# Siverteh/semantic-slam-master

Hardware: AMD Instinct MI355X
Metric: frames/sec extract+match on TUM 640x480; match-index bit-exact vs CPU ref (higher is better)
Workload: dtype f32

## Files before the change

semantic-slam-master_amd/csrc/resample.hip:

```cpp
#include <math.h>

#include <algorithm>

#include "common.h"

namespace {

typedef unsigned u32x4 __attribute__((ext_vector_type(4)));
typedef unsigned u32x2 __attribute__((ext_vector_type(2)));

constexpr int PREC = 22;
constexpr int TX = 64, TY = 16, MAXR = 64;

__device__ __forceinline__ int clip8(int v) {
    v >>= PREC;
    return v < 0 ? 0 : (v > 255 ? 255 : v);
}

__global__ __launch_bounds__(256) void preprocess_kernel(const uint8_t *__restrict__ img, int h, int w, int size,
                                                          const int *__restrict__ bh, const int *__restrict__ ch, int ksh,
                                                          const int *__restrict__ bv, const int *__restrict__ cv, int ksv,
                                                          float *__restrict__ out) {
    __shared__ uint8_t tmp[MAXR][TX][3];
    __shared__ float lut[3][256];
    const int tid = threadIdx.x;
    const long long f = blockIdx.z;
    const int x0 = blockIdx.x * TX, y0 = blockIdx.y * TY;
    const int ty1 = min(y0 + TY, size) - 1;
    const int rmin = bv[2 * y0], rmax = bv[2 * ty1] + bv[2 * ty1 + 1];
    const int nrows = rmax - rmin;
    const uint8_t *src = img + f * h * w * 3;
    {
        const float mean[3] = {0.485f, 0.456f, 0.406f}, sd[3] = {0.229f, 0.224f, 0.225f};
#pragma unroll
        for (int c = 0; c < 3; c++) lut[c][tid] = ((float)tid / 255.0f - mean[c]) / sd[c];
    }
    for (int it = tid; it < nrows * TX; it += 256) {
        const int rr = it / TX, xx = it % TX;
        const int ox = x0 + xx;
        if (ox < size) {
            const int xmin = bh[2 * ox], xn = bh[2 * ox + 1];
            const int *k = ch + (long long)ox * ksh;
            const uint8_t *p = src + ((long long)(rmin + rr) * w + xmin) * 3;
            int s0 = 1 << (PREC - 1), s1 = s0, s2 = s0;
            for (int t = 0; t < xn; t++) {
                const int kk = k[t];
                s0 += p[3 * t] * kk;
                s1 += p[3 * t + 1] * kk;
                s2 += p[3 * t + 2] * kk;
            }
            tmp[rr][xx][0] = (uint8_t)clip8(s0);
            tmp[rr][xx][1] = (uint8_t)clip8(s1);
            tmp[rr][xx][2] = (uint8_t)clip8(s2);
        }
    }
    __syncthreads();
    const long long plane = (long long)size * size;
    for (int it = tid; it < TY * TX * 3; it += 256) {
        const int c = it / (TY * TX), rem = it % (TY * TX), yy = rem / TX, xx = rem % TX;
        const int oy = y0 + yy, ox = x0 + xx;
        if (oy < size && ox < size) {
            const int ymin = bv[2 * oy] - rmin, yn = bv[2 * oy + 1];
            const int *k = cv + (long long)oy * ksv;
            int s = 1 << (PREC - 1);
            for (int t = 0; t < yn; t++) s += tmp[ymin + t][xx][c] * k[t];
            out[(f * 3 + c) * plane + (long long)oy * size + ox] = lut[c][clip8(s)];
        }
    }
}

template <int TAPS, int TYT, int MAXRT, bool PATCH = false>
__global__ __launch_bounds__(256) void preprocess_fast_kernel(const uint8_t *__restrict__ img, unsigned total_bytes, int h, int w,
                                                               int size, const int *__restrict__ bh, const int *__restrict__ ch,
                                                               int ksh, const int *__restrict__ bv, const int *__restrict__ cv,
                                                               int ksv, float *__restrict__ out, int gx, int tiles, int n_frames) {
    __shared__ unsigned tmp[MAXRT][TX];
    __shared__ float lut[3][256];
    const int tid = threadIdx.x;
    const int bq = blockIdx.x >> 3;
    const unsigned f = (unsigned)((bq / tiles) * 8 + (blockIdx.x & 7));
    if ((int)f >= n_frames) return;
    const int tl = bq % tiles;
    const int x0 = (tl % gx) * TX, y0 = (tl / gx) * TYT;
    const int ty1 = min(y0 + TYT, size) - 1;
    const int rmin = bv[2 * y0], rmax = bv[2 * ty1] + bv[2 * ty1 + 1];
    const int nrows = rmax - rmin;
    const __amdgpu_buffer_rsrc_t irs =
        __builtin_amdgcn_make_buffer_rsrc(const_cast<uint8_t *>(img), 0, (int)((total_bytes + 3u) & ~3u), 0x00020000);
    {
        const float mean[3] = {0.485f, 0.456f, 0.406f}, sd[3] = {0.229f, 0.224f, 0.225f};
#pragma unroll
        for (int c = 0; c < 3; c++) lut[c][tid] = ((float)tid / 255.0f - mean[c]) / sd[c];
    }
    const int xx = tid & (TX - 1), q = __builtin_amdgcn_readfirstlane(tid >> 6);
    const int ox = min(x0 + xx, size - 1);
    {
        const int xmin = bh[2 * ox], xn = bh[2 * ox + 1];
        constexpr int NW = (3 * TAPS + 3 + 3) / 4;
        int kh[TAPS];
#pragma unroll
        for (int t = 0; t < TAPS; t++) kh[t] = t < xn ? ch[ox * ksh + t] : 0;
        const unsigned col0 = f * (unsigned)(h * w * 3) + (unsigned)(rmin * w + xmin) * 3u;
        const unsigned rstride = (unsigned)w * 3u;
        constexpr int RB = 3;
        for (int rr0 = q; rr0 < nrows; rr0 += 4 * RB) {
            unsigned wds[RB][8];
            int shv[RB];
#pragma unroll
            for (int i = 0; i < RB; i++) {
                const int rr = min(rr0 + 4 * i, nrows - 1);
                const unsigned b0 = col0 + (unsigned)rr * rstride;
                const int a0 = (int)(b0 & ~3u);
                shv[i] = (int)(b0 & 3u);
                const u32x4 lo = __builtin_amdgcn_raw_buffer_load_b128(irs, a0, 0, 0);
                wds[i][0] = lo[0], wds[i][1] = lo[1], wds[i][2] = lo[2], wds[i][3] = lo[3];
                if constexpr (NW == 5) wds[i][4] = __builtin_amdgcn_raw_buffer_load_b32(irs, a0, 16, 0);
                if constexpr (NW == 6) {
                    const u32x2 hi = __builtin_amdgcn_raw_buffer_load_b64(irs, a0, 16, 0);
                    wds[i][4] = hi[0], wds[i][5] = hi[1];
                }
            }
#pragma unroll
            for (int i = 0; i < RB; i++) {
                const int rr = rr0 + 4 * i;
                if (rr >= nrows) break;
                const int sh = shv[i];
                unsigned al[NW];
#pragma unroll
                for (int j = 0; j < NW - 1; j++) al[j] = __builtin_amdgcn_alignbyte(wds[i][j + 1], wds[i][j], sh);
                al[NW - 1] = wds[i][NW - 1] >> (8 * sh);
                int s0 = 1 << (PREC - 1), s1 = s0, s2 = s0;
#pragma unroll
                for (int t = 0; t < TAPS; t++) {
                    const int o = 3 * t;
                    const int r8 = (al[o >> 2] >> (8 * (o & 3))) & 255;
                    const int g8 = (al[(o + 1) >> 2] >> (8 * ((o + 1) & 3))) & 255;
                    const int b8 = (al[(o + 2) >> 2] >> (8 * ((o + 2) & 3))) & 255;
                    s0 += __mul24(r8, kh[t]);
                    s1 += __mul24(g8, kh[t]);
                    s2 += __mul24(b8, kh[t]);
                }
                tmp[rr][xx] = (unsigned)clip8(s0) | ((unsigned)clip8(s1) << 8) | ((unsigned)clip8(s2) << 16);
            }
        }
    }
    __syncthreads();
    const long long plane = (long long)size * size;
    if (x0 + xx < size) {
#pragma unroll
        for (int j = 0; j < TYT / 4; j++) {
            const int oy = y0 + q * (TYT / 4) + j;
            if (oy < size) {
                const int ymin = bv[2 * oy] - rmin, yn = bv[2 * oy + 1];
                const int *k = cv + oy * ksv;
                int s0 = 1 << (PREC - 1), s1 = s0, s2 = s0;
                for (int t = 0; t < yn; t++) {
                    const unsigned p = tmp[ymin + t][xx];
                    const int kk = k[t];
                    s0 += __mul24((int)(p & 255), kk);
                    s1 += __mul24((int)((p >> 8) & 255), kk);
                    s2 += __mul24((int)((p >> 16) & 255), kk);
                }
                if constexpr (PATCH) {
                    const int G = size >> 4, ox_ = x0 + xx;
                    __bf16 *o = reinterpret_cast<__bf16 *>(out) +
                                (((long long)f * G + (oy >> 4)) * G + (ox_ >> 4)) * 768 + (oy & 15) * 16 + (ox_ & 15);
                    o[0] = (__bf16)lut[0][clip8(s0)];
                    o[256] = (__bf16)lut[1][clip8(s1)];
                    o[512] = (__bf16)lut[2][clip8(s2)];
                } else {
                    float *o = out + (long long)f * 3 * plane + (long long)oy * size + (x0 + xx);
                    o[0] = lut[0][clip8(s0)];
                    o[plane] = lut[1][clip8(s1)];
                    o[2 * plane] = lut[2][clip8(s2)];
                }
            }
        }
    }
}

__global__ __launch_bounds__(256) void intensity_kernel(const uint8_t *__restrict__ img, int h, int w, int size,
                                                         const int *__restrict__ bh, const int *__restrict__ ch, int ksh,
                                                         const int *__restrict__ bv, const int *__restrict__ cv, int ksv,
                                                         const float *__restrict__ kp_pixel, int K, long long total,
                                                         float *__restrict__ out) {
    const long long i = (long long)blockIdx.x * 256 + threadIdx.x;
    if (i >= total) return;
    const long long f = i / K;
    const uint8_t *src = img + f * h * w * 3;
    int X = (int)__builtin_rintf(kp_pixel[2 * i]), Y = (int)__builtin_rintf(kp_pixel[2 * i + 1]);
    X = min(max(X, 0), size - 1);
    Y = min(max(Y, 0), size - 1);
    const int xmin = bh[2 * X], xn = bh[2 * X + 1], ymin = bv[2 * Y], yn = bv[2 * Y + 1];
    const int *kh = ch + (long long)X * ksh, *kv = cv + (long long)Y * ksv;
    int a0 = 1 << (PREC - 1), a1 = a0, a2 = a0;
    for (int ry = 0; ry < yn; ry++) {
        const uint8_t *p = src + ((long long)(ymin + ry) * w + xmin) * 3;
        int s0 = 1 << (PREC - 1), s1 = s0, s2 = s0;
        for (int t = 0; t < xn; t++) {
            const int kk = kh[t];
            s0 += p[3 * t] * kk;
            s1 += p[3 * t + 1] * kk;
            s2 += p[3 * t + 2] * kk;
        }
        const int kk = kv[ry];
        a0 += clip8(s0) * kk;
        a1 += clip8(s1) * kk;
        a2 += clip8(s2) * kk;
    }
    const int R = clip8(a0), Gc = clip8(a1), B = clip8(a2);
    const int L = (R * 19595 + Gc * 38470 + B * 7471 + 0x8000) >> 16;
    out[i] = (float)L / 255.0f;
}

double filt_bilinear(double x) {
    if (x < 0.0) x = -x;
    return x < 1.0 ? 1.0 - x : 0.0;
}
double filt_bicubic(double x) {
    const double a = -0.5;
    if (x < 0.0) x = -x;
    if (x < 1.0) return ((a + 2.0) * x - (a + 3.0)) * x * x + 1;
    if (x < 2.0) return (((x - 5) * x + 8) * x - 4) * a;
    return 0.0;
}

}

extern "C" int sslam_resample_table_host(int in_size, int out_size, int filter, int32_t *bounds, int32_t *coefs,
                                         int coefs_capacity) {
    if (in_size <= 0 || out_size <= 0 || !bounds || !coefs || filter < 0 || filter > 1) return SSLAM_E_INVALID;
    double (*fn)(double) = filter ? filt_bicubic : filt_bilinear;
    const double scale = (double)in_size / out_size;
    double filterscale = scale;
    if (filterscale < 1.0) filterscale = 1.0;
    const double support = (filter ? 2.0 : 1.0) * filterscale;
    const int ksize = (int)ceil(support) * 2 + 1;
    if (ksize > SSLAM_MAX_TAPS) return SSLAM_E_UNSUPPORTED;
    if ((long long)ksize * out_size > coefs_capacity) return SSLAM_E_INVALID;
    double k[SSLAM_MAX_TAPS];
    for (int xx = 0; xx < out_size; xx++) {
        const double center = 0.0 + (xx + 0.5) * scale;
        const double ss = 1.0 / filterscale;
        double ww = 0.0;
        int xmin = (int)(center - support + 0.5);
        if (xmin < 0) xmin = 0;
        int xmax = (int)(center + support + 0.5);
        if (xmax > in_size) xmax = in_size;
        xmax -= xmin;
        int x;
        for (x = 0; x < xmax; x++) {
            const double wgt = fn((x + xmin - center + 0.5) * ss);
            k[x] = wgt;
            ww += wgt;
        }
        for (x = 0; x < xmax; x++)
            if (ww != 0.0) k[x] /= ww;
        for (; x < ksize; x++) k[x] = 0;
        for (x = 0; x < ksize; x++)
            coefs[(long long)xx * ksize + x] =
                k[x] < 0 ? (int32_t)(-0.5 + k[x] * (1 << PREC)) : (int32_t)(0.5 + k[x] * (1 << PREC));
        bounds[2 * xx] = xmin;
        bounds[2 * xx + 1] = xmax;
    }
    return ksize;
}

template <bool PATCH>
static int preprocess_launch(const uint8_t *img, int n, int h, int w, int size, const int32_t *bounds_h, const int32_t *coefs_h,
                             int ksize_h, const int32_t *bounds_v, const int32_t *coefs_v, int ksize_v, void *out_v, void *stream) {
    if (!img || !bounds_h || !coefs_h || !bounds_v || !coefs_v || !out_v || n <= 0 || h <= 0 || w <= 0 || size <= 0)
        return SSLAM_E_INVALID;
    if (ksize_h <= 0 || ksize_v <= 0 || ksize_h > SSLAM_MAX_TAPS || ksize_v > SSLAM_MAX_TAPS) return SSLAM_E_INVALID;
    if (PATCH && size % 16) return SSLAM_E_INVALID;
    if (sslam_misaligned(4, bounds_h, coefs_h, bounds_v, coefs_v) || sslam_misaligned(PATCH ? 2 : 4, out_v)) return SSLAM_E_INVALID;
    if ((long long)(TY * (long long)h + size - 1) / size + ksize_v + 2 > MAXR) return SSLAM_E_UNSUPPORTED;
    const bool tall = (32LL * h + size - 1) / size + ksize_v + 2 <= 64;
    const long long fbytes = (long long)h * w * 3;
    if (fbytes > 0x7fffffffLL) return SSLAM_E_UNSUPPORTED;
    int per_group = (int)std::min<long long>(65535, std::max<long long>(1, 0xfffffff0LL / fbytes));
    if ((fbytes & 3) && per_group >= 4) per_group &= ~3;
    for (int n0 = 0; n0 < n; n0 += per_group) {
        const int ng = std::min(per_group, n - n0);
        const uint8_t *gi = img + (long long)n0 * fbytes;
        const bool aligned = !((uintptr_t)gi & 3);
        float *go = PATCH ? reinterpret_cast<float *>(reinterpret_cast<__bf16 *>(out_v) + (long long)n0 * 3 * size * size)
                          : reinterpret_cast<float *>(out_v) + (long long)n0 * 3 * size * size;
        const unsigned gbytes = (unsigned)(ng * fbytes);
        const dim3 grid((size + TX - 1) / TX, (size + TY - 1) / TY, ng);
        const int gx = (size + TX - 1) / TX, tiles_t = gx * ((size + 31) / 32), tiles_s = gx * ((size + TY - 1) / TY);
        const long long nb_t = (long long)((ng + 7) / 8) * 8 * tiles_t, nb_s = (long long)((ng + 7) / 8) * 8 * tiles_s;
        if (nb_t > 0x7fffffffLL || nb_s > 0x7fffffffLL) return SSLAM_E_UNSUPPORTED;
#define FAST(T)                                                                                                        \
    {                                                                                                                  \
        if (tall)                                                                                                      \
            hipLaunchKernelGGL((preprocess_fast_kernel<T, 32, 64, PATCH>), dim3((unsigned)nb_t), dim3(256), 0, (hipStream_t)stream, gi, gbytes, h, w, \
                               size, bounds_h, coefs_h, ksize_h, bounds_v, coefs_v, ksize_v, go, gx, tiles_t, ng);     \
        else                                                                                                           \
            hipLaunchKernelGGL((preprocess_fast_kernel<T, TY, MAXR, PATCH>), dim3((unsigned)nb_s), dim3(256), 0, (hipStream_t)stream, gi, gbytes, h, w, \
                               size, bounds_h, coefs_h, ksize_h, bounds_v, coefs_v, ksize_v, go, gx, tiles_s, ng);     \
    }
        if (ksize_h <= 3 && aligned)
            FAST(3)
        else if (ksize_h <= 5 && aligned)
            FAST(5)
        else if (ksize_h <= 7 && aligned)
            FAST(7)
        else if (PATCH)
            return SSLAM_E_UNSUPPORTED;
        else
            hipLaunchKernelGGL(preprocess_kernel, grid, dim3(256), 0, (hipStream_t)stream, gi, h, w, size, bounds_h, coefs_h,
                               ksize_h, bounds_v, coefs_v, ksize_v, go);
#undef FAST
    }
    SSLAM_CHECK_LAUNCH();
    return SSLAM_OK;
}

extern "C" int sslam_preprocess_u8(const uint8_t *img, int n, int h, int w, int size, const int32_t *bounds_h,
                                   const int32_t *coefs_h, int ksize_h, const int32_t *bounds_v, const int32_t *coefs_v,
                                   int ksize_v, float *out_chw, void *stream) {
    return preprocess_launch<false>(img, n, h, w, size, bounds_h, coefs_h, ksize_h, bounds_v, coefs_v, ksize_v, out_chw, stream);
}

extern "C" int sslam_preprocess_u8_patches(const uint8_t *img, int n, int h, int w, int size, const int32_t *bounds_h,
                                           const int32_t *coefs_h, int ksize_h, const int32_t *bounds_v, const int32_t *coefs_v,
                                           int ksize_v, void *out_patches_bf16, void *stream) {
    return preprocess_launch<true>(img, n, h, w, size, bounds_h, coefs_h, ksize_h, bounds_v, coefs_v, ksize_v, out_patches_bf16, stream);
}

extern "C" int sslam_keypoint_intensity(const uint8_t *img, int n, int h, int w, int size, const int32_t *bounds_h,
                                        const int32_t *coefs_h, int ksize_h, const int32_t *bounds_v, const int32_t *coefs_v,
                                        int ksize_v, const float *kp_pixel, int K, float *out, void *stream) {
    if (!img || !bounds_h || !coefs_h || !bounds_v || !coefs_v || !kp_pixel || !out || n <= 0 || h <= 0 || w <= 0 ||
        size <= 0 || K <= 0)
        return SSLAM_E_INVALID;
    if (sslam_misaligned(4, bounds_h, coefs_h, bounds_v, coefs_v, kp_pixel, out)) return SSLAM_E_INVALID;
    const long long total = (long long)n * K;
    hipLaunchKernelGGL(intensity_kernel, dim3((unsigned)((total + 255) / 256)), dim3(256), 0, (hipStream_t)stream, img, h, w,
                       size, bounds_h, coefs_h, ksize_h, bounds_v, coefs_v, ksize_v, kp_pixel, K, total, out);
    SSLAM_CHECK_LAUNCH();
    return SSLAM_OK;
}
```

Measured before the change: 58200.

## Add templated buffer-load keypoint intensity kernel and nontemporal preprocess stores

Adds a templated intensity kernel for small filter sizes. It fetches each source row with wide raw buffer loads, unpacks the bytes with alignbyte, and fully unrolls both filter passes, replacing per-byte global loads inside dynamic loops. The preprocess kernel gains asm barriers that keep the batched row loads in registers so they stay issued ahead of use, and its f32 output now uses nontemporal stores to avoid polluting the cache. The fast path is taken only when kernel sizes, image alignment and sizes allow; otherwise the old kernel still runs. This adds code size and template variants.

```diff
diff --git a/semantic-slam-master_amd/csrc/resample.hip b/semantic-slam-master_amd/csrc/resample.hip
--- a/semantic-slam-master_amd/csrc/resample.hip
+++ b/semantic-slam-master_amd/csrc/resample.hip
@@ -120,6 +120,10 @@
                     wds[i][4] = hi[0], wds[i][5] = hi[1];
                 }
             }
+#pragma unroll
+            for (int i = 0; i < RB; i++)
+#pragma unroll
+                for (int j = 0; j < NW; j++) asm volatile("" : "+v"(wds[i][j]));
 #pragma unroll
             for (int i = 0; i < RB; i++) {
                 const int rr = rr0 + 4 * i;
@@ -170,9 +174,9 @@
                     o[512] = (__bf16)lut[2][clip8(s2)];
                 } else {
                     float *o = out + (long long)f * 3 * plane + (long long)oy * size + (x0 + xx);
-                    o[0] = lut[0][clip8(s0)];
-                    o[plane] = lut[1][clip8(s1)];
-                    o[2 * plane] = lut[2][clip8(s2)];
+                    __builtin_nontemporal_store(lut[0][clip8(s0)], o);
+                    __builtin_nontemporal_store(lut[1][clip8(s1)], o + plane);
+                    __builtin_nontemporal_store(lut[2][clip8(s2)], o + 2 * plane);
                 }
             }
         }
@@ -210,6 +214,70 @@
     }
     const int R = clip8(a0), Gc = clip8(a1), B = clip8(a2);
     const int L = (R * 19595 + Gc * 38470 + B * 7471 + 0x8000) >> 16;
+    out[i] = (float)L / 255.0f;
+}
+
+template <int TAPS, int VT>
+__global__ __launch_bounds__(256) void intensity_fast_kernel(const uint8_t *__restrict__ img, unsigned total_bytes, int h, int w,
+                                                              int size, const int *__restrict__ bh, const int *__restrict__ ch,
+                                                              int ksh, const int *__restrict__ bv, const int *__restrict__ cv,
+                                                              int ksv, const float *__restrict__ kp_pixel, int K, int total,
+                                                              float *__restrict__ out) {
+    const int i = blockIdx.x * 256 + threadIdx.x;
+    if (i >= total) return;
+    const unsigned f = (unsigned)i / (unsigned)K;
+    const __amdgpu_buffer_rsrc_t irs =
+        __builtin_amdgcn_make_buffer_rsrc(const_cast<uint8_t *>(img), 0, (int)((total_bytes + 3u) & ~3u), 0x00020000);
+    int X = (int)__builtin_rintf(kp_pixel[2 * (size_t)i]), Y = (int)__builtin_rintf(kp_pixel[2 * (size_t)i + 1]);
+    X = min(max(X, 0), size - 1);
+    Y = min(max(Y, 0), size - 1);
+    const int xmin = bh[2 * X], xn = bh[2 * X + 1], ymin = bv[2 * Y], yn = bv[2 * Y + 1];
+    constexpr int NW = (3 * TAPS + 3 + 3) / 4;
+    const unsigned col0 = f * (unsigned)(h * w * 3) + (unsigned)(ymin * w + xmin) * 3u;
+    const unsigned rstride = (unsigned)w * 3u;
+    unsigned wds[VT][8];
+#pragma unroll
+    for (int ry = 0; ry < VT; ry++) {
+#pragma unroll
+        for (int j = 0; j < NW; j++) wds[ry][j] = 0;
+        if (ry < yn) {
+            const int a0 = (int)((col0 + (unsigned)ry * rstride) & ~3u);
+            const u32x4 lo = __builtin_amdgcn_raw_buffer_load_b128(irs, a0, 0, 0);
+            wds[ry][0] = lo[0], wds[ry][1] = lo[1], wds[ry][2] = lo[2], wds[ry][3] = lo[3];
+            if constexpr (NW == 5) wds[ry][4] = __builtin_amdgcn_raw_buffer_load_b32(irs, a0, 16, 0);
+            if constexpr (NW == 6) {
+                const u32x2 hi = __builtin_amdgcn_raw_buffer_load_b64(irs, a0, 16, 0);
+                wds[ry][4] = hi[0], wds[ry][5] = hi[1];
+            }
+        }
+    }
+    int kh[TAPS], kv[VT];
+#pragma unroll
+    for (int t = 0; t < TAPS; t++) kh[t] = t < xn ? ch[X * ksh + min(t, ksh - 1)] : 0;
+#pragma unroll
+    for (int t = 0; t < VT; t++) kv[t] = t < yn ? cv[Y * ksv + min(t, ksv - 1)] : 0;
+    int a0 = 1 << (PREC - 1), a1 = a0, a2 = a0;
+#pragma unroll
+    for (int ry = 0; ry < VT; ry++) {
+        const int sh = (int)((col0 + (unsigned)ry * rstride) & 3u);
+        unsigned al[NW];
+#pragma unroll
+        for (int j = 0; j < NW - 1; j++) al[j] = __builtin_amdgcn_alignbyte(wds[ry][j + 1], wds[ry][j], sh);
+        al[NW - 1] = wds[ry][NW - 1] >> (8 * sh);
+        int s0 = 1 << (PREC - 1), s1 = s0, s2 = s0;
+#pragma unroll
+        for (int t = 0; t < TAPS; t++) {
+            const int o = 3 * t;
+            s0 += __mul24((int)((al[o >> 2] >> (8 * (o & 3))) & 255), kh[t]);
+            s1 += __mul24((int)((al[(o + 1) >> 2] >> (8 * ((o + 1) & 3))) & 255), kh[t]);
+            s2 += __mul24((int)((al[(o + 2) >> 2] >> (8 * ((o + 2) & 3))) & 255), kh[t]);
+        }
+        a0 += __mul24(clip8(s0), kv[ry]);
+        a1 += __mul24(clip8(s1), kv[ry]);
+        a2 += __mul24(clip8(s2), kv[ry]);
+    }
+    const int R = clip8(a0), Gc = clip8(a1), B = clip8(a2);
+    const int L = (__mul24(R, 19595) + __mul24(Gc, 38470) + __mul24(B, 7471) + 0x8000) >> 16;
     out[i] = (float)L / 255.0f;
 }
 
@@ -336,9 +404,32 @@
         size <= 0 || K <= 0)
         return SSLAM_E_INVALID;
     if (sslam_misaligned(4, bounds_h, coefs_h, bounds_v, coefs_v, kp_pixel, out)) return SSLAM_E_INVALID;
-    const long long total = (long long)n * K;
-    hipLaunchKernelGGL(intensity_kernel, dim3((unsigned)((total + 255) / 256)), dim3(256), 0, (hipStream_t)stream, img, h, w,
-                       size, bounds_h, coefs_h, ksize_h, bounds_v, coefs_v, ksize_v, kp_pixel, K, total, out);
+    const long long total = (long long)n * K, bytes = (long long)n * h * w * 3;
+    const dim3 grid((unsigned)((total + 255) / 256));
+    const bool fast = ksize_h <= 7 && ksize_v <= 7 && !((uintptr_t)img & 3) && bytes <= 0xfffffff0LL && total <= 0x7fffff00LL;
+#define FASTI(T, V)                                                                                                    \
+    hipLaunchKernelGGL((intensity_fast_kernel<T, V>), grid, dim3(256), 0, (hipStream_t)stream, img, (unsigned)bytes, h, w, size, \
+                       bounds_h, coefs_h, ksize_h, bounds_v, coefs_v, ksize_v, kp_pixel, K, (int)total, out)
+#define FASTV(T)                                                                                                       \
+    {                                                                                                                  \
+        if (ksize_v <= 3)                                                                                              \
+            FASTI(T, 3);                                                                                               \
+        else if (ksize_v <= 5)                                                                                         \
+            FASTI(T, 5);                                                                                               \
+        else                                                                                                           \
+            FASTI(T, 7);                                                                                               \
+    }
+    if (fast && ksize_h <= 3)
+        FASTV(3)
+    else if (fast && ksize_h <= 5)
+        FASTV(5)
+    else if (fast)
+        FASTV(7)
+    else
+        hipLaunchKernelGGL(intensity_kernel, grid, dim3(256), 0, (hipStream_t)stream, img, h, w, size, bounds_h, coefs_h,
+                           ksize_h, bounds_v, coefs_v, ksize_v, kp_pixel, K, total, out);
+#undef FASTV
+#undef FASTI
     SSLAM_CHECK_LAUNCH();
     return SSLAM_OK;
 }
```

Result: faster. 58870 (median of 6 runs) (+1.1%).
